# zama-ai/verifiable-fhe-paper

Measured on AMD Instinct MI355X. Metric: vPBS proofs/sec at N=1024 (1/2/4/8 GPU); prover ms/proof vs CPU baseline, higher is better.
Workload: dtype u64; 1 GPU; N=1024 vPBS as IVC chain (BASELINE config 2; verified_pbs ivc_based_vpbs.rs:159-386) via vpbs_ivc_prove_pbs; step = 1 chained proof of the cyclic circuit (2^16 rows) per chain; chains_per_gpu=8, parallelism=replicas, witness=host

## Files before the change

### verifiable-fhe-paper_amd/csrc/hash.hip

```cpp
#include <cstdlib>

#include <algorithm>
#include "kernels.h"
#include "poseidon.h"

namespace vpbs {
namespace {
constexpr unsigned THREADS = 256;

template <bool SAMPLE>
__global__ void __launch_bounds__(THREADS)
leaf_hash_kernel(const u64* __restrict__ lde, unsigned ncols, size_t n_leaves, size_t col_stride, u64* __restrict__ digests,
                 u64* __restrict__ clock_sample) {
    const size_t j = blockIdx.x * (size_t)THREADS + threadIdx.x;
    if (j >= n_leaves) return;
    const bool sample = SAMPLE && clock_sample != nullptr && blockIdx.x == gridDim.x / 2 && threadIdx.x == 0;
    u64 c0 = 0, r0 = 0;
    if (sample) {
        r0 = __builtin_amdgcn_s_memrealtime();
        c0 = __builtin_amdgcn_s_memtime();
    }
    u64 s[12];
#pragma unroll
    for (int i = 0; i < 12; ++i) s[i] = 0;
    if (ncols <= 4) {
#pragma unroll
        for (int k = 0; k < 4; ++k)
            if ((unsigned)k < ncols) s[k] = lde[k * col_stride + j];
    } else {
        u64 nxt[8];
#pragma unroll
        for (int k = 0; k < 8; ++k)
            if ((unsigned)k < ncols) s[k] = lde[(size_t)k * col_stride + j];
        for (unsigned c0 = 0;; c0 += 8) {
            if (c0 + 8 < ncols) {
#pragma unroll
                for (int k = 0; k < 8; ++k)
                    if (c0 + 8 + k < ncols) nxt[k] = lde[(size_t)(c0 + 8 + k) * col_stride + j];
            }
            const bool more = poseidon::permute_sponge(s, ncols - c0, [&](unsigned n) {
#pragma unroll
                for (int k = 0; k < 8; ++k)
                    if ((unsigned)k < n) s[k] = nxt[k];
            });
            if (!more) break;
        }
#pragma unroll
        for (int k = 0; k < 4; ++k) s[k] = gl::canon(s[k]);
    }
    ulonglong2* d = reinterpret_cast<ulonglong2*>(digests + 4 * j);
    d[0] = make_ulonglong2(s[0], s[1]);
    d[1] = make_ulonglong2(s[2], s[3]);
    if (sample) {
        clock_sample[0] = __builtin_amdgcn_s_memtime() - c0;
        clock_sample[1] = __builtin_amdgcn_s_memrealtime() - r0;
    }
}

__global__ void __launch_bounds__(THREADS)
fri_leaf_hash_kernel(const u64* __restrict__ v0, const u64* __restrict__ v1, size_t n_leaves, unsigned arity_bits,
                     u64* __restrict__ digests) {
    const size_t l = blockIdx.x * (size_t)THREADS + threadIdx.x;
    if (l >= n_leaves) return;
    const unsigned arity = 1u << arity_bits;
    const size_t base = l << arity_bits;
    u64 s[12];
#pragma unroll
    for (int i = 0; i < 12; ++i) s[i] = 0;
    if (2 * arity <= 4) {
#pragma unroll
        for (int m = 0; m < 2; ++m)
            if ((unsigned)m < arity) { s[2 * m] = v0[base + m]; s[2 * m + 1] = v1[base + m]; }
    } else {
#pragma unroll
        for (int k = 0; k < 4; ++k)
            if ((unsigned)k < arity) { s[2 * k] = v0[base + k]; s[2 * k + 1] = v1[base + k]; }
        for (unsigned m0 = 0;; m0 += 4) {
            const bool more = poseidon::permute_sponge(s, 2 * (arity - m0), [&](unsigned n) {
#pragma unroll
                for (int k = 0; k < 4; ++k)
                    if (2 * (unsigned)k < n) { s[2 * k] = v0[base + m0 + 4 + k]; s[2 * k + 1] = v1[base + m0 + 4 + k]; }
            });
            if (!more) break;
        }
#pragma unroll
        for (int k = 0; k < 4; ++k) s[k] = gl::canon(s[k]);
    }
    ulonglong2* d = reinterpret_cast<ulonglong2*>(digests + 4 * l);
    d[0] = make_ulonglong2(s[0], s[1]);
    d[1] = make_ulonglong2(s[2], s[3]);
}

__global__ void __launch_bounds__(THREADS)
merkle_level_kernel(const u64* __restrict__ children, u64* __restrict__ parents, size_t n_parents) {
    const size_t i = blockIdx.x * (size_t)THREADS + threadIdx.x;
    if (i >= n_parents) return;
    const ulonglong2* c = reinterpret_cast<const ulonglong2*>(children + 8 * i);
    const ulonglong2 a = c[0], b = c[1], e = c[2], f = c[3];
    u64 s[12] = {a.x, a.y, b.x, b.y, e.x, e.y, f.x, f.y, 0, 0, 0, 0};
// ... 38 lines not shown
            const bool live = i < m;
            u64 x = 0;
            if (live && l < 8) x = k == 0 ? src[8 * i + l] : buf[(k - 1) & 1][8 * i + l];
            x = poseidon::permute_wide(x, lds + g * poseidon::WIDE_LDS_WORDS, l);
            if (live && l < 4) {
                dst[4 * i + l] = x;
                buf[k & 1][4 * i + l] = x;
            }
        }
        __syncthreads();
    }
}

__global__ void __launch_bounds__(THREADS)
fri_leaf_hash_wide_kernel(const u64* __restrict__ v0, const u64* __restrict__ v1, size_t n_leaves, unsigned arity_bits,
                          u64* __restrict__ digests) {
    __shared__ u64 lds[(THREADS / poseidon::WIDE_LANES) * poseidon::WIDE_LDS_WORDS];
    const unsigned l = threadIdx.x & 15, g = threadIdx.x >> 4;
    const size_t leaf = blockIdx.x * (size_t)(THREADS / 16) + g;
    const bool live = leaf < n_leaves;
    const unsigned n_elems = 2u << arity_bits;
    const size_t base = leaf << arity_bits;
    u64 x = 0;
    for (unsigned e0 = 0; e0 < n_elems; e0 += 8) {
        const unsigned e = e0 + l;
        if (l < 8 && e < n_elems && live) x = ((e & 1) ? v1 : v0)[base + (e >> 1)];
        x = poseidon::permute_wide(x, lds + g * poseidon::WIDE_LDS_WORDS, l);
    }
    if (live && l < 4) digests[4 * leaf + l] = x;
}

__global__ void __launch_bounds__(THREADS) permute_batch_kernel(u64* states, size_t n) {
    const size_t i = blockIdx.x * (size_t)THREADS + threadIdx.x;
    if (i >= n) return;
    u64 s[12];
#pragma unroll
    for (int k = 0; k < 12; ++k) s[k] = states[12 * i + k];
    poseidon::permute(s);
#pragma unroll
    for (int k = 0; k < 12; ++k) states[12 * i + k] = s[k];
}

__global__ void __launch_bounds__(THREADS)
hash_rows_kernel(const u64* __restrict__ rows, size_t n, unsigned len, u64* __restrict__ out) {
    const size_t i = blockIdx.x * (size_t)THREADS + threadIdx.x;
    if (i >= n) return;
    const u64* row = rows + i * len;
    u64 s[12];
#pragma unroll
    for (int k = 0; k < 12; ++k) s[k] = 0;
#pragma unroll
    for (int k = 0; k < 8; ++k)
        if ((unsigned)k < len) s[k] = row[k];
    for (unsigned c0 = 0;; c0 += 8) {
        const bool more = poseidon::permute_sponge(s, len - c0, [&](unsigned n) {
#pragma unroll
            for (int k = 0; k < 8; ++k)
                if ((unsigned)k < n) s[k] = row[c0 + 8 + k];
        });
        if (!more) break;
    }
#pragma unroll
    for (int k = 0; k < 4; ++k) out[4 * i + k] = gl::canon(s[k]);
}

struct PowState {
    u64 s[12];
};

__global__ void __launch_bounds__(THREADS)
pow_search_kernel(PowState st, unsigned pos, unsigned pow_bits, u64 start, u64 count, u64 stride, unsigned long long* result) {
    const u64 i = blockIdx.x * (u64)THREADS + threadIdx.x;
    if (i >= stride) return;
    for (u64 off = i; off < count; off += stride) {
        const u64 cand = start + off;
        if (__atomic_load_n(result, __ATOMIC_RELAXED) < cand) return;
        u64 s[12];
#pragma unroll
        for (int k = 0; k < 12; ++k) s[k] = (unsigned)k == pos ? cand : st.s[k];
        poseidon::permute_residues(s);
        if (pow_bits == 0 || (gl::canon(s[7]) >> (64 - pow_bits)) == 0) {
            atomicMin(result, (unsigned long long)cand);
            return;
        }
    }
}
}

void launch_leaf_hash(hipStream_t s, const u64* lde, unsigned ncols, size_t n_leaves, size_t col_stride, u64* digests, u64* clock_sample) {
    if (clock_sample)
        hipLaunchKernelGGL(leaf_hash_kernel<true>, dim3((n_leaves + THREADS - 1) / THREADS), dim3(THREADS), 0, s, lde, ncols, n_leaves,
                           col_stride, digests, clock_sample);
    else
        hipLaunchKernelGGL(leaf_hash_kernel<false>, dim3((n_leaves + THREADS - 1) / THREADS), dim3(THREADS), 0, s, lde, ncols, n_leaves,
                           col_stride, digests, clock_sample);
}
Tuning Tuning::from_env() {
    Tuning t;
    if (const char* e = getenv("VPBS_WIDE_THRESHOLD")) t.wide_threshold = t.fri_leaf_wide_threshold = (size_t)strtoull(e, nullptr, 10);
    if (const char* e = getenv("VPBS_FRI_LEAF_WIDE_THRESHOLD")) t.fri_leaf_wide_threshold = (size_t)strtoull(e, nullptr, 10);
    if (const char* e = getenv("VPBS_MERKLE_CLIMB")) t.merkle_climb = atoi(e) != 0;
    if (const char* e = getenv("VPBS_GATES_FUSED")) t.gates_fused = atoi(e) != 0;
    if (const char* e = getenv("VPBS_GATE_ITEMS")) t.gate_items = (unsigned)std::max(1, atoi(e));
    if (const char* e = getenv("VPBS_GATES_TILE")) t.gates_tile = atoi(e) != 0;
    return t;
}

void launch_fri_leaf_hash(hipStream_t s, const Tuning& tune, const u64* v0, const u64* v1, size_t n_leaves, unsigned arity_bits, u64* digests) {
    if (n_leaves <= tune.fri_leaf_wide_threshold && (2u << arity_bits) > 4) {
        hipLaunchKernelGGL(fri_leaf_hash_wide_kernel, dim3((unsigned)((n_leaves * 16 + THREADS - 1) / THREADS)), dim3(THREADS), 0, s, v0,
                           v1, n_leaves, arity_bits, digests);
        return;
    }
    hipLaunchKernelGGL(fri_leaf_hash_kernel, dim3((n_leaves + THREADS - 1) / THREADS), dim3(THREADS), 0, s, v0, v1, n_leaves,
// ... 49 lines not shown
```

### verifiable-fhe-paper_amd/csrc/poseidon.h

```cpp
#pragma once
#include "gl.h"

namespace poseidon {
using gl::u32;
using gl::u64;

constexpr int WIDTH = 12, RATE = 8, N_ROUNDS = 30, HALF_FULL = 4, N_PARTIAL = 22;

static const u64 RC_HOST[372] = {
#include "poseidon_constants.inc"
};
#if defined(__HIPCC__)
static __constant__ u64 RC_DEV[372] = {
#include "poseidon_constants.inc"
};
#endif

#include "poseidon_partial_groups.inc"
static const PartialGroup PG_HOST[7] = POSEIDON_PARTIAL_GROUPS_INIT;
#if defined(__HIPCC__)
static __constant__ PartialGroup PG_DEV[7] = POSEIDON_PARTIAL_GROUPS_INIT;
#endif
GL_HD const PartialGroup& partial_group(int g) {
#if defined(__HIP_DEVICE_COMPILE__)
// ... 175 lines not shown
            "v_mad_u64_u32 %0, vcc, %10, 39, %0\n\t"
            "v_mad_u64_u32 %1, vcc, %22, 39, %1\n\t"
            "v_mad_u64_u32 %0, vcc, %11, 18, %0\n\t"
            "v_mad_u64_u32 %1, vcc, %23, 18, %1\n\t"
            "v_mad_u64_u32 %0, vcc, %12, 34, %0\n\t"
            "v_mad_u64_u32 %1, vcc, %24, 34, %1\n\t"
            "v_mad_u64_u32 %0, vcc, %13, 20, %0\n\t"
            "v_mad_u64_u32 %1, vcc, %25, 20, %1"
                : "=&v"(acc_lo), "=&v"(acc_hi)
                : POSEIDON_ROW_OPERANDS
                : "vcc");
    }
}
#endif

GL_HD void mds_add_const(u64* s, const u64* kc) {
    u32 lo[12], hi[12];
#pragma unroll
    for (int i = 0; i < 12; ++i) {
        lo[i] = (u32)s[i];
        hi[i] = (u32)(s[i] >> 32);
    }
#pragma unroll
    for (int r = 0; r < 12; ++r) {
        u64 acc_lo, acc_hi;
#if defined(__HIP_DEVICE_COMPILE__)
        u32 xl[12], xh[12];
#pragma unroll
        for (int i = 0; i < 12; ++i) {
            xl[i] = lo[(i + r) % 12];
            xh[i] = hi[(i + r) % 12];
        }
        if (kc) {
            if (r == 0) mds_row<true, true>(xl, xh, kc[r], acc_lo, acc_hi);
            else mds_row<false, true>(xl, xh, kc[r], acc_lo, acc_hi);
        } else {
            if (r == 0) mds_row<true, false>(xl, xh, 0, acc_lo, acc_hi);
            else mds_row<false, false>(xl, xh, 0, acc_lo, acc_hi);
        }
#else
        const u32 C[12] = {17, 15, 41, 16, 2, 28, 13, 13, 39, 18, 34, 20};
        const u64 k = kc ? kc[r] : 0;
        acc_lo = (u32)k, acc_hi = k >> 32;
        for (int i = 0; i < 12; ++i) {
            const u32 c = r == 0 && i == 0 ? C[0] + 8 : C[i];
            acc_lo += (u64)lo[(i + r) % 12] * c;
            acc_hi += (u64)hi[(i + r) % 12] * c;
        }
#endif
        s[r] = fold96(acc_lo, acc_hi);
    }
}

#if defined(__HIP_DEVICE_COMPILE__)
template <unsigned M1>
__device__ __forceinline__ void group_row(u32 d3l, u32 d3h, u32 d2l, u32 d2h, u32 m2, u64 k, const u32* xl, const u32* xh, const u32* m3, u64& acc_lo,
                                          u64& acc_hi) {
    static_assert(M1 <= 64, "inline constant");
    asm("s_mov_b32 s82, %43\n\t"
        "s_and_b32 s83, %44, 0x03ffffff\n\t"
        "s_and_b32 s84, %44, 0xfc000000\n\t"
        "s_mov_b32 s85, 0\n\t"
        "v_mad_u64_u32 %0, vcc, %2, %45, s[82:83]\n\t"
        "v_mad_u64_u32 %1, vcc, %3, %45, s[84:85]\n\t"
        "v_mad_u64_u32 %0, vcc, %4, %6, %0\n\t"
        "v_mad_u64_u32 %1, vcc, %5, %6, %1\n\t"
        "v_mad_u64_u32 %0, vcc, %7, %31, %0\n\t"
        "v_mad_u64_u32 %1, vcc, %19, %31, %1\n\t"
        "v_mad_u64_u32 %0, vcc, %8, %32, %0\n\t"
        "v_mad_u64_u32 %1, vcc, %20, %32, %1\n\t"
        "v_mad_u64_u32 %0, vcc, %9, %33, %0\n\t"
        "v_mad_u64_u32 %1, vcc, %21, %33, %1\n\t"
        "v_mad_u64_u32 %0, vcc, %10, %34, %0\n\t"
        "v_mad_u64_u32 %1, vcc, %22, %34, %1\n\t"
        "v_mad_u64_u32 %0, vcc, %11, %35, %0\n\t"
        "v_mad_u64_u32 %1, vcc, %23, %35, %1\n\t"
        "v_mad_u64_u32 %0, vcc, %12, %36, %0\n\t"
        "v_mad_u64_u32 %1, vcc, %24, %36, %1\n\t"
        "v_mad_u64_u32 %0, vcc, %13, %37, %0\n\t"
        "v_mad_u64_u32 %1, vcc, %25, %37, %1\n\t"
        "v_mad_u64_u32 %0, vcc, %14, %38, %0\n\t"
        "v_mad_u64_u32 %1, vcc, %26, %38, %1\n\t"
        "v_mad_u64_u32 %0, vcc, %15, %39, %0\n\t"
        "v_mad_u64_u32 %1, vcc, %27, %39, %1\n\t"
        "v_mad_u64_u32 %0, vcc, %16, %40, %0\n\t"
        "v_mad_u64_u32 %1, vcc, %28, %40, %1\n\t"
        "v_mad_u64_u32 %0, vcc, %17, %41, %0\n\t"
        "v_mad_u64_u32 %1, vcc, %29, %41, %1\n\t"
        "v_mad_u64_u32 %0, vcc, %18, %42, %0\n\t"
        "v_mad_u64_u32 %1, vcc, %30, %42, %1"
        : "=&v"(acc_lo), "=&v"(acc_hi)
        : "v"(d3l), "v"(d3h), "v"(d2l), "v"(d2h), "s"(m2),
          "v"(xl[0]), "v"(xl[1]), "v"(xl[2]), "v"(xl[3]), "v"(xl[4]), "v"(xl[5]), "v"(xl[6]), "v"(xl[7]), "v"(xl[8]), "v"(xl[9]), "v"(xl[10]),
          "v"(xl[11]),
          "v"(xh[0]), "v"(xh[1]), "v"(xh[2]), "v"(xh[3]), "v"(xh[4]), "v"(xh[5]), "v"(xh[6]), "v"(xh[7]), "v"(xh[8]), "v"(xh[9]), "v"(xh[10]),
          "v"(xh[11]),
          "s"(m3[0]), "s"(m3[1]), "s"(m3[2]), "s"(m3[3]), "s"(m3[4]), "s"(m3[5]), "s"(m3[6]), "s"(m3[7]), "s"(m3[8]), "s"(m3[9]), "s"(m3[10]),
          "s"(m3[11]),
          "s"((u32)k), "s"((u32)(k >> 32)), "n"(M1)
        : "vcc", "scc", "s82", "s83", "s84", "s85");
}
template <int I> struct GroupRow {
    static __device__ __forceinline__ void run(u64* s, const u64* kv, const u32* lo, const u32* hi, u32 d2l, u32 d2h, u32 d3l, u32 d3h) {
        u32 m3[12];
#pragma unroll
        for (int j = 0; j < 12; ++j) m3[j] = MDS3[I][j];
// ... 18 lines not shown
        hi[j] = (u32)(s[j] >> 32);
    }
    u64 a_lo = (u32)k2, a_hi = k2 >> 32;
#pragma unroll
    for (int j = 0; j < 12; ++j) {
        a_lo += (u64)lo[j] * MDS1[0][j];
        a_hi += (u64)hi[j] * MDS1[0][j];
    }
    u64 x2 = fold96(a_lo, a_hi);
    if (GATE || x_out) {
        x2 = gl::canon(x2);
        x_out[0] = x2;
    }
    const u64 d2 = gl::sub_a(sbox(GATE ? w[1] : x2), x2);
    const u32 d2l = (u32)d2, d2h = (u32)(d2 >> 32);
    u64 b_lo = (u32)k3, b_hi = k3 >> 32;
#pragma unroll
    for (int j = 0; j < 12; ++j) {
        b_lo += (u64)lo[j] * MDS2[0][j];
        b_hi += (u64)hi[j] * MDS2[0][j];
    }
    b_lo += (u64)d2l * MDS1[0][0];
    b_hi += (u64)d2h * MDS1[0][0];
    u64 x3 = fold96(b_lo, b_hi);
    if (GATE || x_out) {
        x3 = gl::canon(x3);
        x_out[1] = x3;
    }
    const u64 d3 = gl::sub_a(sbox(GATE ? w[2] : x3), x3);
    const u32 d3l = (u32)d3, d3h = (u32)(d3 >> 32);
#if defined(__HIP_DEVICE_COMPILE__)
    GroupRow<0>::run(s, kv, lo, hi, d2l, d2h, d3l, d3h);
#else
#pragma unroll
    for (int i = 0; i < 12; ++i) {
        const u64 k = kv[i];
        u64 acc_lo = (u32)k, acc_hi = k >> 32;
#pragma unroll
        for (int j = 0; j < 12; ++j) {
            acc_lo += (u64)lo[j] * MDS3[i][j];
            acc_hi += (u64)hi[j] * MDS3[i][j];
        }
        acc_lo += (u64)d2l * MDS2[i][0] + (u64)d3l * MDS1[i][0];
        acc_hi += (u64)d2h * MDS2[i][0] + (u64)d3h * MDS1[i][0];
        s[i] = fold96(acc_lo, acc_hi);
    }
#endif
}
template <bool GATE> GL_HD void partial_group3_core(u64* s, int g, const u64* w, u64* x_out) {
    partial_group3_core<GATE>(s, partial_group(g), w, x_out);
}
GL_HD void partial_group3(u64* s, int g) { partial_group3_core<false>(s, g, nullptr, nullptr); }

static const ClosingGroup CG_HOST = POSEIDON_CLOSING_GROUP_INIT;
#if defined(__HIPCC__)
static __constant__ ClosingGroup CG_DEV = POSEIDON_CLOSING_GROUP_INIT;
#endif
GL_HD const ClosingGroup& closing_group(int z) {
#if defined(__HIP_DEVICE_COMPILE__)
    return (&CG_DEV)[z];
#else
    return (&CG_HOST)[z];
#endif
}
#if defined(__HIP_DEVICE_COMPILE__)
__device__ __forceinline__ void halves_sum(const u32* xl, const u32* xh, u64& sum_lo, u64& sum_hi) {
    asm("v_mad_u64_u32 %0, vcc, %2, 1, 0\n\t"
        "v_mad_u64_u32 %1, vcc, %14, 1, 0\n\t"
        "v_mad_u64_u32 %0, vcc, %3, 1, %0\n\t"
        "v_mad_u64_u32 %1, vcc, %15, 1, %1\n\t"
        "v_mad_u64_u32 %0, vcc, %4, 1, %0\n\t"
        "v_mad_u64_u32 %1, vcc, %16, 1, %1\n\t"
        "v_mad_u64_u32 %0, vcc, %5, 1, %0\n\t"
        "v_mad_u64_u32 %1, vcc, %17, 1, %1\n\t"
        "v_mad_u64_u32 %0, vcc, %6, 1, %0\n\t"
        "v_mad_u64_u32 %1, vcc, %18, 1, %1\n\t"
        "v_mad_u64_u32 %0, vcc, %7, 1, %0\n\t"
        "v_mad_u64_u32 %1, vcc, %19, 1, %1\n\t"
        "v_mad_u64_u32 %0, vcc, %8, 1, %0\n\t"
        "v_mad_u64_u32 %1, vcc, %20, 1, %1\n\t"
        "v_mad_u64_u32 %0, vcc, %9, 1, %0\n\t"
        "v_mad_u64_u32 %1, vcc, %21, 1, %1\n\t"
        "v_mad_u64_u32 %0, vcc, %10, 1, %0\n\t"
        "v_mad_u64_u32 %1, vcc, %22, 1, %1\n\t"
        "v_mad_u64_u32 %0, vcc, %11, 1, %0\n\t"
        "v_mad_u64_u32 %1, vcc, %23, 1, %1\n\t"
        "v_mad_u64_u32 %0, vcc, %12, 1, %0\n\t"
        "v_mad_u64_u32 %1, vcc, %24, 1, %1\n\t"
        "v_mad_u64_u32 %0, vcc, %13, 1, %0\n\t"
        "v_mad_u64_u32 %1, vcc, %25, 1, %1"
        : "=&v"(sum_lo), "=&v"(sum_hi)
        : POSEIDON_ROW_OPERANDS
        : "vcc");
}
template <unsigned M1>
__device__ __forceinline__ void closing_row(u32 d4l, u32 d4h, u32 d3l, u32 d3h, u32 m2, u32 d2l, u32 d2h, u32 m3, u32 tl, u32 th, u32 base, u64 k,
                                            const u32* xl, const u32* xh, const u32* n, u64& acc_lo, u64& acc_hi) {
    static_assert(M1 <= 64, "inline constant");
    asm("s_mov_b32 s82, %49\n\t"
        "s_and_b32 s83, %50, 0x03ffffff\n\t"
        "s_and_b32 s84, %50, 0xfc000000\n\t"
        "s_mov_b32 s85, 0\n\t"
        "v_mad_u64_u32 %0, vcc, %2, %51, s[82:83]\n\t"
        "v_mad_u64_u32 %1, vcc, %3, %51, s[84:85]\n\t"
        "v_mad_u64_u32 %0, vcc, %4, %6, %0\n\t"
        "v_mad_u64_u32 %1, vcc, %5, %6, %1\n\t"
        "v_mad_u64_u32 %0, vcc, %7, %9, %0\n\t"
        "v_mad_u64_u32 %1, vcc, %8, %9, %1\n\t"
        "v_mad_u64_u32 %0, vcc, %10, %12, %0\n\t"
        "v_mad_u64_u32 %1, vcc, %11, %12, %1\n\t"
        "v_mad_u64_u32 %0, vcc, %13, %37, %0\n\t"
        "v_mad_u64_u32 %1, vcc, %25, %37, %1\n\t"
        "v_mad_u64_u32 %0, vcc, %14, %38, %0\n\t"
        "v_mad_u64_u32 %1, vcc, %26, %38, %1\n\t"
        "v_mad_u64_u32 %0, vcc, %15, %39, %0\n\t"
        "v_mad_u64_u32 %1, vcc, %27, %39, %1\n\t"
        "v_mad_u64_u32 %0, vcc, %16, %40, %0\n\t"
// ... 63 lines not shown
    u64 b_lo = (u32)k3, b_hi = k3 >> 32;
#pragma unroll
    for (int j = 0; j < 12; ++j) {
        b_lo += (u64)lo[j] * MDS2[0][j];
        b_hi += (u64)hi[j] * MDS2[0][j];
    }
    b_lo += (u64)d2l * MDS1[0][0];
    b_hi += (u64)d2h * MDS1[0][0];
    const u64 x3 = fold96(b_lo, b_hi);
    const u64 d3 = gl::sub_a(sbox(WIRES ? w[2] : x3), x3);
    const u32 d3l = (u32)d3, d3h = (u32)(d3 >> 32);
    u64 c_lo = (u32)k4, c_hi = k4 >> 32;
#pragma unroll
    for (int j = 0; j < 12; ++j) {
        c_lo += (u64)lo[j] * MDS3[0][j];
        c_hi += (u64)hi[j] * MDS3[0][j];
    }
    c_lo += (u64)d2l * MDS2[0][0] + (u64)d3l * MDS1[0][0];
    c_hi += (u64)d2h * MDS2[0][0] + (u64)d3h * MDS1[0][0];
    const u64 x4 = fold96(c_lo, c_hi);
    const u64 d4 = gl::sub_a(sbox(WIRES ? w[3] : x4), x4);
    const u32 d4l = (u32)d4, d4h = (u32)(d4 >> 32);
    u64 t_lo, t_hi;
#if defined(__HIP_DEVICE_COMPILE__)
    halves_sum(lo, hi, t_lo, t_hi);
#else
    t_lo = 0, t_hi = 0;
    for (int j = 0; j < 12; ++j) {
        t_lo += lo[j];
        t_hi += hi[j];
    }
#endif
    const u64 t = fold96(t_lo, t_hi);
    const u32 tl = (u32)t, th = (u32)(t >> 32);
#if defined(__HIP_DEVICE_COMPILE__)
    ClosingRow<0>::run(s, kv, lo, hi, d2l, d2h, d3l, d3h, d4l, d4h, tl, th);
#else
#pragma unroll
    for (int i = 0; i < 12; ++i) {
        const u64 k = kv[i];
        u64 acc_lo = (u32)k, acc_hi = k >> 32;
#pragma unroll
        for (int j = 0; j < 12; ++j) {
            acc_lo += (u64)lo[j] * (MDS4[i][j] - MDS4_BASE[i]);
            acc_hi += (u64)hi[j] * (MDS4[i][j] - MDS4_BASE[i]);
        }
        acc_lo += (u64)tl * MDS4_BASE[i] + (u64)d2l * MDS3[i][0] + (u64)d3l * MDS2[i][0] + (u64)d4l * MDS1[i][0];
        acc_hi += (u64)th * MDS4_BASE[i] + (u64)d2h * MDS3[i][0] + (u64)d3h * MDS2[i][0] + (u64)d4h * MDS1[i][0];
        s[i] = fold96(acc_lo, acc_hi);
    }
#endif
}
GL_HD void closing_group4(u64* s, int z = 0) { closing_group4_core<false>(s, closing_group(z), nullptr); }

GL_HD void permute_head(u64* s) {
#if defined(__HIP_DEVICE_COMPILE__)
    int z;
    asm volatile("s_mov_b32 %0, 0" : "=s"(z));
#else
    constexpr int z = 0;
#endif
#pragma unroll
    for (int i = 0; i < 12; ++i) s[i] = gl::add_nc(s[i], rc(z + i));
    for (int r = 0; r < HALF_FULL; ++r) {
        u64 kc[12];
#pragma unroll
        for (int i = 0; i < 12; ++i) kc[i] = rc(12 * (r + 1) + i);
#pragma unroll
        for (int i = 0; i < 12; i += 2) sbox2(s[i], s[i + 1]);
        mds_add_const(s, kc);
    }
    {
        for (int g = 0; g < 6; ++g) partial_group3(s, g);
    }
    {
#if defined(__HIP_DEVICE_COMPILE__)
        int z4;
        asm volatile("s_mov_b32 %0, 0" : "=s"(z4));
#else
        constexpr int z4 = 0;
#endif
        closing_group4(s, z4);
    }
    for (int r = HALF_FULL + N_PARTIAL; r < N_ROUNDS - 1; ++r) {
        u64 kc[12];
#pragma unroll
        for (int i = 0; i < 12; ++i) kc[i] = rc(12 * (r + 1) + i);
#pragma unroll
        for (int i = 0; i < 12; i += 2) sbox2(s[i], s[i + 1]);
        mds_add_const(s, kc);
    }
#pragma unroll
    for (int i = 0; i < 12; i += 2) sbox2(s[i], s[i + 1]);
}
struct HeadHalves {
    u32 lo[12], hi[12];
};
GL_HD HeadHalves head_halves(const u64* s) {
    HeadHalves h;
#pragma unroll
    for (int i = 0; i < 12; ++i) {
        h.lo[i] = (u32)s[i];
        h.hi[i] = (u32)(s[i] >> 32);
    }
    return h;
}
template <int FIRST, int COUNT> GL_HD void last_rows(u64* s, const HeadHalves& h) {
    static_assert(FIRST >= 0 && COUNT > 0 && FIRST + COUNT <= 12, "rows of a width-12 state");
#pragma unroll
    for (int r = FIRST; r < FIRST + COUNT; ++r) {
        u64 acc_lo, acc_hi;
#if defined(__HIP_DEVICE_COMPILE__)
        u32 xl[12], xh[12];
#pragma unroll
        for (int i = 0; i < 12; ++i) {
            xl[i] = h.lo[(i + r) % 12];
            xh[i] = h.hi[(i + r) % 12];
        }
        if (r == 0) mds_row<true, false>(xl, xh, 0, acc_lo, acc_hi);
        else mds_row<false, false>(xl, xh, 0, acc_lo, acc_hi);
#else
        const u32 C[12] = {17, 15, 41, 16, 2, 28, 13, 13, 39, 18, 34, 20};
        acc_lo = 0, acc_hi = 0;
        for (int i = 0; i < 12; ++i) {
            const u32 c = r == 0 && i == 0 ? C[0] + 8 : C[i];
            acc_lo += (u64)h.lo[(i + r) % 12] * c;
            acc_hi += (u64)h.hi[(i + r) % 12] * c;
        }
#endif
        s[r] = fold96(acc_lo, acc_hi);
    }
}

GL_HD void permute_residues(u64* s) {
    permute_head(s);
    last_rows<0, 12>(s, head_halves(s));
}
template <class Absorb> GL_HD bool permute_sponge(u64* s, unsigned remaining, Absorb&& absorb) {
    permute_head(s);
#if defined(__HIP_DEVICE_COMPILE__)
    asm volatile("" : "+s"(remaining));
#endif
    const HeadHalves h = head_halves(s);
    if (remaining <= 8) {
        last_rows<0, 4>(s, h);
        return false;
    }
    last_rows<8, 4>(s, h);
    if (remaining < 16) {
        last_rows<0, 8>(s, h);
        absorb(remaining - 8);
    } else {
        absorb(8u);
    }
    return true;
}
GL_HD void permute_digest(u64* s) {
    permute_head(s);
    last_rows<0, 4>(s, head_halves(s));
}
GL_HD void permute(u64* s) {
    permute_residues(s);
#pragma unroll
    for (int i = 0; i < 12; ++i) s[i] = gl::canon(s[i]);
}

#if defined(__HIPCC__)
constexpr int WIDE_LANES = 16, WIDE_LDS_WORDS = 48;
__device__ __forceinline__ u64 permute_wide(u64 x, u64* sh, unsigned l) {
    constexpr u32 C[12] = {17, 15, 41, 16, 2, 28, 13, 13, 39, 18, 34, 20};
    const unsigned row = l < 12 ? l : 0;
    u32 m3[12];
#pragma unroll
    for (int j = 0; j < 12; ++j) m3[j] = MDS3[row][j];
    const u32 m2c = MDS2[row][0], m1c = MDS1[row][0];
    x = gl::add_nc(x, rc(row));
    u64 kplain[9], kgroup[7];
#pragma unroll
    for (int i = 0; i < 9; ++i) {
        const int r = i < 4 ? i : HALF_FULL + N_PARTIAL - 1 + (i - 4);
        kplain[i] = r + 1 < N_ROUNDS ? rc(12 * (r + 1) + row) : 0;
    }
#pragma unroll
    for (int g = 0; g < 7; ++g) kgroup[g] = partial_group(g).kvec[row];
    auto plain_round = [&](u64 k, bool full) {
        if (full || l == 0) x = sbox_ilp(x);
        __builtin_amdgcn_fence(__ATOMIC_ACQ_REL, "wavefront");
        if (l < 12) {
            sh[l] = x;
            sh[l + 12] = x;
        }
        __builtin_amdgcn_fence(__ATOMIC_ACQ_REL, "wavefront");
        u64 al[3] = {(u32)k, 0, 0}, ah[3] = {k >> 32, 0, 0};
#pragma unroll
        for (int i = 0; i < 12; ++i) {
            const u64 v = sh[row + i];
            al[i % 3] += (u64)(u32)v * C[i];
            ah[i % 3] += (v >> 32) * C[i];
        }
        if (l == 0) {
            al[1] += (u64)(u32)x * 8u;
            ah[1] += (x >> 32) * 8u;
        }
        x = fold96(al[0] + al[1] + al[2], ah[0] + ah[1] + ah[2]);
    };
#pragma unroll
    for (int i = 0; i < HALF_FULL; ++i) plain_round(kplain[i], true);
#pragma unroll
    for (int g = 0; g < 7; ++g) {
        const PartialGroup& G = partial_group(g);
        const u64 k2 = G.k2, k3 = G.k3, kv = kgroup[g];
// ... 50 lines not shown
```

### verifiable-fhe-paper_amd/csrc/poseidon_partial_groups.inc

```
static constexpr unsigned MDS1[12][12] = {
    {25, 15, 41, 16, 2, 28, 13, 13, 39, 18, 34, 20},
    {20, 17, 15, 41, 16, 2, 28, 13, 13, 39, 18, 34},
    {34, 20, 17, 15, 41, 16, 2, 28, 13, 13, 39, 18},
    {18, 34, 20, 17, 15, 41, 16, 2, 28, 13, 13, 39},
    {39, 18, 34, 20, 17, 15, 41, 16, 2, 28, 13, 13},
    {13, 39, 18, 34, 20, 17, 15, 41, 16, 2, 28, 13},
    {13, 13, 39, 18, 34, 20, 17, 15, 41, 16, 2, 28},
    {28, 13, 13, 39, 18, 34, 20, 17, 15, 41, 16, 2},
    {2, 28, 13, 13, 39, 18, 34, 20, 17, 15, 41, 16},
    {16, 2, 28, 13, 13, 39, 18, 34, 20, 17, 15, 41},
    {41, 16, 2, 28, 13, 13, 39, 18, 34, 20, 17, 15},
    {15, 41, 16, 2, 28, 13, 13, 39, 18, 34, 20, 17},
};
static constexpr unsigned MDS2[12][12] = {
    {5642, 5952, 4914, 5368, 6238, 5356, 5302, 6080, 5870, 4880, 6818, 5364},
    {5364, 5306, 5832, 4586, 5240, 6222, 5132, 5198, 5976, 5558, 4736, 6546},
    {6818, 5204, 5306, 5832, 4586, 5240, 6222, 5132, 5198, 5976, 5558, 4736},
    {4880, 6546, 5204, 5306, 5832, 4586, 5240, 6222, 5132, 5198, 5976, 5558},
    {5870, 4736, 6546, 5204, 5306, 5832, 4586, 5240, 6222, 5132, 5198, 5976},
    {6080, 5558, 4736, 6546, 5204, 5306, 5832, 4586, 5240, 6222, 5132, 5198},
    {5302, 5976, 5558, 4736, 6546, 5204, 5306, 5832, 4586, 5240, 6222, 5132},
    {5356, 5198, 5976, 5558, 4736, 6546, 5204, 5306, 5832, 4586, 5240, 6222},
    {6238, 5132, 5198, 5976, 5558, 4736, 6546, 5204, 5306, 5832, 4586, 5240},
    {5368, 6222, 5132, 5198, 5976, 5558, 4736, 6546, 5204, 5306, 5832, 4586},
    {4914, 5240, 6222, 5132, 5198, 5976, 5558, 4736, 6546, 5204, 5306, 5832},
    {5952, 4586, 5240, 6222, 5132, 5198, 5976, 5558, 4736, 6546, 5204, 5306},
};
static constexpr unsigned MDS3[12][12] = {
    {1525684, 1438872, 1418228, 1480072, 1422580, 1420320, 1506604, 1416584, 1444108, 1476584, 1436396, 1411808},
    {1411808, 1437100, 1395776, 1375900, 1435272, 1376884, 1375744, 1464500, 1372416, 1394724, 1440536, 1380428},
    {1436396, 1370256, 1445852, 1393568, 1373884, 1442568, 1375940, 1377200, 1473028, 1371072, 1401092, 1440536},
    {1476584, 1379388, 1372080, 1437004, 1389504, 1377372, 1436824, 1374276, 1379280, 1465012, 1371072, 1394724},
    {1444108, 1439776, 1390020, 1371168, 1435324, 1397952, 1377396, 1439008, 1384572, 1379280, 1473028, 1372416},
    {1416584, 1393404, 1439360, 1378892, 1366384, 1437612, 1390568, 1374692, 1439008, 1374276, 1377200, 1464500},
    {1506604, 1367736, 1396108, 1436760, 1377436, 1369088, 1436052, 1390568, 1377396, 1436824, 1375940, 1375744},
    {1420320, 1465780, 1375360, 1395428, 1435544, 1383500, 1369088, 1437612, 1397952, 1377372, 1442568, 1376884},
    {1422580, 1373904, 1463076, 1366432, 1391876, 1435544, 1377436, 1366384, 1435324, 1389504, 1373884, 1435272},
    {1480072, 1374324, 1378912, 1464468, 1366432, 1395428, 1436760, 1378892, 1371168, 1437004, 1393568, 1375900},
    {1418228, 1439872, 1385852, 1378912, 1463076, 1375360, 1396108, 1439360, 1390020, 1372080, 1445852, 1395776},
    {1438872, 1375140, 1439872, 1374324, 1373904, 1465780, 1367736, 1393404, 1439776, 1379388, 1370256, 1437100},
};
struct PartialGroup { unsigned long long kvec[12]; unsigned long long k2, k3; };
#define POSEIDON_PARTIAL_GROUPS_INIT { \
    {{0xfe4e957d77fda909ULL, 0x3847b97fc56907d4ULL, 0x0a1b7d0f67cfc238ULL, 0xc414e2bfdddee685ULL, 0x2717635d4d088529ULL, 0x40491e688918641bULL, 0x560b36b7f479beafULL, 0xda7596d883b42c13ULL, 0xd8b7b84768d7843aULL, 0x733c8ebad2af2843ULL, 0x8f92cf546fb87dcdULL, 0x6081e328cce022cdULL}, 0x7131aa45268d7d8cULL, 0xff1b1d52a1d8bb71ULL}, \
    {{0xd119def35a30b511ULL, 0x6785e26657976c04ULL, 0x4c85e0f0e498b80aULL, 0x09b2f2891e72516eULL, 0xe8b03d4698e681aaULL, 0x943c922624343e1eULL, 0x490186833eb8ae37ULL, 0xab44b27eb875bd36ULL, 0xf675f2dac0d2b4adULL, 0x0735fb41dfb4abedULL, 0xec6d46a358c64e19ULL, 0x71183a53d224b708ULL}, 0x7159cd30c3ac118eULL, 0x50c17f4e8bc2a7b5ULL}, \
    {{0x54eafd5e8c0ef61dULL, 0xfe06121da3b5b838ULL, 0x0ef385ebd5715833ULL, 0x61a0a6709460c24fULL, 0xc6a94f23db583ec5ULL, 0x3bb2b2e7586de7c0ULL, 0xae705460e5c84923ULL, 0x20d3881afc6b4518ULL, 0x0cc8cad7bd42cc91ULL, 0x2f4efc14e6672a3fULL, 0xbd0bae3dce7d33d9ULL, 0xe258d7e08e8bd3b8ULL}, 0x30a4680593258387ULL, 0x875e5dbdfa0a1b6bULL}, \
    {{0x2d5e442f2de9aea9ULL, 0x1c4170bab0c28bfeULL, 0xfbd4c3193585cc9eULL, 0x596c7a704f8f3f2aULL, 0xceef25ac926d22dfULL, 0x54ac7c785c0f4ff3ULL, 0x7c55c7d7dcf17873ULL, 0xdc9e8e30b8caaa76ULL, 0x5f7782ff3c614fcaULL, 0x4d4176f913e999feULL, 0xa5ce4725b751e6f8ULL, 0xf5d10a11c024a67aULL}, 0x775005982d74d7f7ULL, 0xe6b47ac7fadcceacULL}, \
    {{0x5fdb985df94d5f34ULL, 0x3e6e5ea6969897f8ULL, 0x39e628df805fb70aULL, 0x8dabe2e2b77195acULL, 0xbaae0d3685531a78ULL, 0x836cc600e5475c67ULL, 0x6a1cf353276fa432ULL, 0x35f461ba3266eef6ULL, 0xde7afd90ec069d5dULL, 0x5f578ca248341311ULL, 0x606e5560329a8266ULL, 0x88eb2c660628a242ULL}, 0xdd611f1000c17442ULL, 0x82c8567c0dad8fd2ULL}, \
    {{0xbb167cb775013794ULL, 0x87befcca0b83baffULL, 0x44d6d7813828842aULL, 0x3452da396d341fccULL, 0x94b4a33439d5d74fULL, 0xbba4cb68152c5ab5ULL, 0x8798e5ade84f4253ULL, 0x6268ed55dec1949dULL, 0x6084862992f892baULL, 0x3748775cf424ec3fULL, 0x19197866793dcb9fULL, 0xf9cbdd030cb77598ULL}, 0xe89cd854d5d01d33ULL, 0xfc39f87979d52a85ULL}, \
    {{0x3eec5e59c10be794ULL, 0x921c7513b98436fdULL, 0x8f4003a60c2aa013ULL, 0x9f75572964678803ULL, 0x3e9495107539a5e1ULL, 0x617c7acbc1db897fULL, 0x43530ee6648e366aULL, 0xce98d5d027df583fULL, 0xb6d54eb500e52d7cULL, 0x553fc8926939fc86ULL, 0x30cfbdbb7b960c7fULL, 0xfa93f9bc7bf7381aULL}, 0xde122bebe9a39368ULL, 0x5718e9d82e27faebULL}, \
}
static constexpr unsigned MDS4[12][12] = {
    {381558488, 369288112, 374533544, 369959168, 369454632, 373358944, 370265576, 368886800, 375007320, 369607648, 370277912, 373854368},
    {373854368, 357623704, 358824096, 362304040, 357790720, 359163384, 361468960, 358453864, 358738272, 362530840, 358873600, 358107144},
    {370277912, 363385904, 359530600, 358628928, 362580520, 359632512, 359263656, 362413968, 360578840, 358445408, 364635672, 358873600},
    {369607648, 357841672, 363242464, 357426104, 357304992, 362611176, 357965408, 358508792, 362402336, 358324552, 358445408, 362530840},
    {375007320, 358891216, 359772456, 363367680, 358082088, 359247008, 363011304, 359184368, 360706264, 362402336, 360578840, 358738272},
    {368886800, 362336792, 358838416, 357739464, 361725808, 357942552, 357503856, 362032872, 359184368, 358508792, 362413968, 358453864},
    {370265576, 357418192, 363216664, 357590848, 357148184, 362702816, 357138904, 357503856, 363011304, 357965408, 359263656, 361468960},
    {373358944, 358888936, 358959456, 362859992, 357846656, 358765576, 362702816, 357942552, 359247008, 362611176, 359632512, 359163384},
    {369454632, 360921296, 359059288, 357057728, 361200024, 357846656, 357148184, 361725808, 358082088, 357304992, 362580520, 357790720},
    {369959168, 358531384, 362427136, 358297672, 357057728, 362859992, 357590848, 357739464, 363367680, 357426104, 358628928, 362304040},
    {374533544, 359211952, 360256728, 362427136, 359059288, 358959456, 363216664, 358838416, 359772456, 363242464, 359530600, 358824096},
    {369288112, 362193128, 359211952, 358531384, 360921296, 358888936, 357418192, 362336792, 358891216, 357841672, 363385904, 357623704},
};
static constexpr unsigned MDS4_BASE[12] = {368886800, 357623704, 358445408, 357304992, 358082088, 357503856, 357138904, 357846656, 357057728, 357057728, 358824096, 357418192};
struct ClosingGroup { unsigned long long kvec[12]; unsigned long long k2, k3, k4; };
#define POSEIDON_CLOSING_GROUP_INIT {{0xdc95f1ec2eb3244dULL, 0x287446500cf761ecULL, 0x8b0d2dd37a860ec8ULL, 0xc5f62d4d042a566cULL, 0xc10a7d2f956ec953ULL, 0x435e1e18c9743ccdULL, 0x9f0b0c6ef65b1a78ULL, 0x776d3954f3c88850ULL, 0x0dea5a60554b6830ULL, 0x53ae1b1b1753161bULL, 0x82f6927bdb4b82b4ULL, 0x5b176968ca1309e4ULL}, 0xde122bebe9a39368ULL, 0x5718e9d82e27faebULL, 0x3eec5e59c10be794ULL}
```

Baseline: 0.2134 vPBS proofs/s.

## Specialize Poseidon first round for zero capacity and regroup partial rounds by four

```diff
diff --git a/verifiable-fhe-paper_amd/csrc/hash.hip b/verifiable-fhe-paper_amd/csrc/hash.hip
--- a/verifiable-fhe-paper_amd/csrc/hash.hip
+++ b/verifiable-fhe-paper_amd/csrc/hash.hip
@@ -32,19 +32,20 @@
 #pragma unroll
         for (int k = 0; k < 8; ++k)
             if ((unsigned)k < ncols) s[k] = lde[(size_t)k * col_stride + j];
-        for (unsigned c0 = 0;; c0 += 8) {
-            if (c0 + 8 < ncols) {
-#pragma unroll
-                for (int k = 0; k < 8; ++k)
-                    if (c0 + 8 + k < ncols) nxt[k] = lde[(size_t)(c0 + 8 + k) * col_stride + j];
-            }
-            const bool more = poseidon::permute_sponge(s, ncols - c0, [&](unsigned n) {
+        poseidon::sponge_from_zero(
+            s, ncols,
+            [&](unsigned c) {
+                if (c < ncols) {
+#pragma unroll
+                    for (int k = 0; k < 8; ++k)
+                        if (c + k < ncols) nxt[k] = lde[(size_t)(c + k) * col_stride + j];
+                }
+            },
+            [&](unsigned, unsigned n) {
 #pragma unroll
                 for (int k = 0; k < 8; ++k)
                     if ((unsigned)k < n) s[k] = nxt[k];
             });
-            if (!more) break;
-        }
 #pragma unroll
         for (int k = 0; k < 4; ++k) s[k] = gl::canon(s[k]);
     }
@@ -189,14 +190,13 @@
 #pragma unroll
     for (int k = 0; k < 8; ++k)
         if ((unsigned)k < len) s[k] = row[k];
-    for (unsigned c0 = 0;; c0 += 8) {
-        const bool more = poseidon::permute_sponge(s, len - c0, [&](unsigned n) {
+    poseidon::sponge_from_zero(
+        s, len, [](unsigned) {},
+        [&](unsigned w, unsigned n) {
 #pragma unroll
             for (int k = 0; k < 8; ++k)
-                if ((unsigned)k < n) s[k] = row[c0 + 8 + k];
+                if ((unsigned)k < n) s[k] = row[w + k];
         });
-        if (!more) break;
-    }
 #pragma unroll
     for (int k = 0; k < 4; ++k) out[4 * i + k] = gl::canon(s[k]);
 }
diff --git a/verifiable-fhe-paper_amd/csrc/poseidon.h b/verifiable-fhe-paper_amd/csrc/poseidon.h
--- a/verifiable-fhe-paper_amd/csrc/poseidon.h
+++ b/verifiable-fhe-paper_amd/csrc/poseidon.h
@@ -251,6 +251,78 @@
     }
 }
 
+static const u64 ZC_K1_HOST[12] = POSEIDON_ZERO_CAPACITY_K1_INIT;
+#if defined(__HIPCC__)
+static __constant__ u64 ZC_K1_DEV[12] = POSEIDON_ZERO_CAPACITY_K1_INIT;
+#endif
+GL_HD u64 zero_capacity_k1(int i) {
+#if defined(__HIP_DEVICE_COMPILE__)
+    return ZC_K1_DEV[i];
+#else
+    return ZC_K1_HOST[i];
+#endif
+}
+#if defined(__HIP_DEVICE_COMPILE__)
+template <int R> __device__ __forceinline__ void mds_row8(const u32* xl, const u32* xh, u64 k, u64& acc_lo, u64& acc_hi) {
+    asm("s_mov_b32 s82, %18\n\t"
+        "s_and_b32 s83, %19, 0x03ffffff\n\t"
+        "s_and_b32 s84, %19, 0xfc000000\n\t"
+        "s_mov_b32 s85, 0\n\t"
+        "v_mad_u64_u32 %0, vcc, %2, %20, s[82:83]\n\t"
+        "v_mad_u64_u32 %1, vcc, %10, %20, s[84:85]\n\t"
+        "v_mad_u64_u32 %0, vcc, %3, %21, %0\n\t"
+        "v_mad_u64_u32 %1, vcc, %11, %21, %1\n\t"
+        "v_mad_u64_u32 %0, vcc, %4, %22, %0\n\t"
+        "v_mad_u64_u32 %1, vcc, %12, %22, %1\n\t"
+        "v_mad_u64_u32 %0, vcc, %5, %23, %0\n\t"
+        "v_mad_u64_u32 %1, vcc, %13, %23, %1\n\t"
+        "v_mad_u64_u32 %0, vcc, %6, %24, %0\n\t"
+        "v_mad_u64_u32 %1, vcc, %14, %24, %1\n\t"
+        "v_mad_u64_u32 %0, vcc, %7, %25, %0\n\t"
+        "v_mad_u64_u32 %1, vcc, %15, %25, %1\n\t"
+        "v_mad_u64_u32 %0, vcc, %8, %26, %0\n\t"
+        "v_mad_u64_u32 %1, vcc, %16, %26, %1\n\t"
+        "v_mad_u64_u32 %0, vcc, %9, %27, %0\n\t"
+        "v_mad_u64_u32 %1, vcc, %17, %27, %1"
+        : "=&v"(acc_lo), "=&v"(acc_hi)
+        : "v"(xl[0]), "v"(xl[1]), "v"(xl[2]), "v"(xl[3]), "v"(xl[4]), "v"(xl[5]), "v"(xl[6]), "v"(xl[7]),
+          "v"(xh[0]), "v"(xh[1]), "v"(xh[2]), "v"(xh[3]), "v"(xh[4]), "v"(xh[5]), "v"(xh[6]), "v"(xh[7]),
+          "s"((u32)k), "s"((u32)(k >> 32)),
+          "n"(MDS1[R][0]), "n"(MDS1[R][1]), "n"(MDS1[R][2]), "n"(MDS1[R][3]), "n"(MDS1[R][4]), "n"(MDS1[R][5]), "n"(MDS1[R][6]),
+          "n"(MDS1[R][7])
+        : "vcc", "scc", "s82", "s83", "s84", "s85");
+}
+template <int R> struct MdsRow8 {
+    static_assert(MDS1[R][0] <= 64 && MDS1[R][7] <= 64, "inline constants");
+    static __device__ __forceinline__ void run(u64* s, const u64* kc, const u32* lo, const u32* hi) {
+        u64 acc_lo, acc_hi;
+        mds_row8<R>(lo, hi, kc[R], acc_lo, acc_hi);
+        s[R] = fold96(acc_lo, acc_hi);
+        if constexpr (R + 1 < 12) MdsRow8<R + 1>::run(s, kc, lo, hi);
+    }
+};
+#endif
+GL_HD void mds8_add_const(u64* s, const u64* kc) {
+    u32 lo[8], hi[8];
+#pragma unroll
+    for (int j = 0; j < 8; ++j) {
+        lo[j] = (u32)s[j];
+        hi[j] = (u32)(s[j] >> 32);
+    }
+#if defined(__HIP_DEVICE_COMPILE__)
+    MdsRow8<0>::run(s, kc, lo, hi);
+#else
+    for (int i = 0; i < 12; ++i) {
+        u64 acc_lo = (u32)kc[i], acc_hi = kc[i] >> 32;
+        for (int j = 0; j < 8; ++j) {
+            acc_lo += (u64)lo[j] * MDS1[i][j];
+            acc_hi += (u64)hi[j] * MDS1[i][j];
+        }
+        s[i] = fold96(acc_lo, acc_hi);
+    }
+#endif
+}
+
 #if defined(__HIP_DEVICE_COMPILE__)
 template <unsigned M1>
 __device__ __forceinline__ void group_row(u32 d3l, u32 d3h, u32 d2l, u32 d2h, u32 m2, u64 k, const u32* xl, const u32* xh, const u32* m3, u64& acc_lo,
@@ -375,17 +447,18 @@
 }
 GL_HD void partial_group3(u64* s, int g) { partial_group3_core<false>(s, g, nullptr, nullptr); }
 
-static const ClosingGroup CG_HOST = POSEIDON_CLOSING_GROUP_INIT;
+static const ClosingGroup G4_HOST[POSEIDON_N_GROUPS4] = POSEIDON_GROUPS4_INIT;
 #if defined(__HIPCC__)
-static __constant__ ClosingGroup CG_DEV = POSEIDON_CLOSING_GROUP_INIT;
-#endif
-GL_HD const ClosingGroup& closing_group(int z) {
-#if defined(__HIP_DEVICE_COMPILE__)
-    return (&CG_DEV)[z];
-#else
-    return (&CG_HOST)[z];
-#endif
-}
+static __constant__ ClosingGroup G4_DEV[POSEIDON_N_GROUPS4] = POSEIDON_GROUPS4_INIT;
+#endif
+GL_HD const ClosingGroup& group4_constants(int g) {
+#if defined(__HIP_DEVICE_COMPILE__)
+    return G4_DEV[g];
+#else
+    return G4_HOST[g];
+#endif
+}
+GL_HD const ClosingGroup& closing_group(int z) { return group4_constants(POSEIDON_N_GROUPS4 - 1 + z); }
 #if defined(__HIP_DEVICE_COMPILE__)
 __device__ __forceinline__ void halves_sum(const u32* xl, const u32* xh, u64& sum_lo, u64& sum_hi) {
     asm("v_mad_u64_u32 %0, vcc, %2, 1, 0\n\t"
@@ -555,8 +628,14 @@
 #endif
 }
 GL_HD void closing_group4(u64* s, int z = 0) { closing_group4_core<false>(s, closing_group(z), nullptr); }
-
-GL_HD void permute_head(u64* s) {
+GL_HD void partial_group4(u64* s, int g) {
+    closing_group4_core<false>(s, group4_constants(g), nullptr);
+#if defined(__HIP_DEVICE_COMPILE__)
+    asm volatile("" : "+v"(s[0]), "+v"(s[1]), "+v"(s[2]), "+v"(s[3]), "+v"(s[4]), "+v"(s[5]), "+v"(s[6]), "+v"(s[7]), "+v"(s[8]), "+v"(s[9]), "+v"(s[10]), "+v"(s[11]));
+#endif
+}
+
+GL_HD void head_first_constants(u64* s) {
 #if defined(__HIP_DEVICE_COMPILE__)
     int z;
     asm volatile("s_mov_b32 %0, 0" : "=s"(z));
@@ -565,7 +644,34 @@
 #endif
 #pragma unroll
     for (int i = 0; i < 12; ++i) s[i] = gl::add_nc(s[i], rc(z + i));
-    for (int r = 0; r < HALF_FULL; ++r) {
+}
+GL_HD void head_zero_capacity_round(u64* s) {
+    u64 kc[12];
+#pragma unroll
+    for (int i = 0; i < 12; ++i) kc[i] = zero_capacity_k1(i);
+#pragma unroll
+    for (int i = 0; i < 8; ++i) s[i] = gl::add_nc(s[i], rc(i));
+#pragma unroll
+    for (int i = 0; i < 8; i += 2) sbox2(s[i], s[i + 1]);
+    mds8_add_const(s, kc);
+}
+GL_HD void partial_rounds(u64* s) {
+#pragma nounroll
+    for (int g = 0; g < POSEIDON_N_GROUPS4 - 1; ++g) partial_group4(s, g);
+#pragma nounroll
+    for (int g = 4; g < 6; ++g) partial_group3(s, g);
+    {
+#if defined(__HIP_DEVICE_COMPILE__)
+        int z4;
+        asm volatile("s_mov_b32 %0, 0" : "=s"(z4));
+#else
+        constexpr int z4 = 0;
+#endif
+        closing_group4(s, z4);
+    }
+}
+GL_HD void head_from_round(u64* s, int r0) {
+    for (int r = r0; r < HALF_FULL; ++r) {
         u64 kc[12];
 #pragma unroll
         for (int i = 0; i < 12; ++i) kc[i] = rc(12 * (r + 1) + i);
@@ -573,18 +679,7 @@
         for (int i = 0; i < 12; i += 2) sbox2(s[i], s[i + 1]);
         mds_add_const(s, kc);
     }
-    {
-        for (int g = 0; g < 6; ++g) partial_group3(s, g);
-    }
-    {
-#if defined(__HIP_DEVICE_COMPILE__)
-        int z4;
-        asm volatile("s_mov_b32 %0, 0" : "=s"(z4));
-#else
-        constexpr int z4 = 0;
-#endif
-        closing_group4(s, z4);
-    }
+    partial_rounds(s);
     for (int r = HALF_FULL + N_PARTIAL; r < N_ROUNDS - 1; ++r) {
         u64 kc[12];
 #pragma unroll
@@ -595,6 +690,15 @@
     }
 #pragma unroll
     for (int i = 0; i < 12; i += 2) sbox2(s[i], s[i + 1]);
+}
+template <bool ZERO_CAPACITY = false> GL_HD void permute_head(u64* s) {
+    if constexpr (ZERO_CAPACITY) {
+        head_zero_capacity_round(s);
+        head_from_round(s, 1);
+    } else {
+        head_first_constants(s);
+        head_from_round(s, 0);
+    }
 }
 struct HeadHalves {
     u32 lo[12], hi[12];
@@ -639,8 +743,7 @@
     permute_head(s);
     last_rows<0, 12>(s, head_halves(s));
 }
-template <class Absorb> GL_HD bool permute_sponge(u64* s, unsigned remaining, Absorb&& absorb) {
-    permute_head(s);
+template <class Absorb> GL_HD bool sponge_rows(u64* s, unsigned remaining, Absorb&& absorb) {
 #if defined(__HIP_DEVICE_COMPILE__)
     asm volatile("" : "+s"(remaining));
 #endif
@@ -658,8 +761,23 @@
     }
     return true;
 }
+template <bool FIRST = false, class Absorb> GL_HD bool permute_sponge(u64* s, unsigned remaining, Absorb&& absorb) {
+    permute_head<FIRST>(s);
+    return sponge_rows(s, remaining, absorb);
+}
+template <class Prefetch, class Absorb> GL_HD void sponge_from_zero(u64* s, unsigned n_words, Prefetch&& prefetch, Absorb&& absorb) {
+    head_zero_capacity_round(s);
+    int r0 = 1;
+    for (unsigned w = 0;; w += 8) {
+        prefetch(w + 8);
+        head_from_round(s, r0);
+        if (!sponge_rows(s, n_words - w, [&](unsigned n) { absorb(w + 8, n); })) break;
+        head_first_constants(s);
+        r0 = 0;
+    }
+}
 GL_HD void permute_digest(u64* s) {
-    permute_head(s);
+    permute_head<true>(s);
     last_rows<0, 4>(s, head_halves(s));
 }
 GL_HD void permute(u64* s) {
diff --git a/verifiable-fhe-paper_amd/csrc/poseidon_partial_groups.inc b/verifiable-fhe-paper_amd/csrc/poseidon_partial_groups.inc
--- a/verifiable-fhe-paper_amd/csrc/poseidon_partial_groups.inc
+++ b/verifiable-fhe-paper_amd/csrc/poseidon_partial_groups.inc
@@ -66,4 +66,11 @@
 };
 static constexpr unsigned MDS4_BASE[12] = {368886800, 357623704, 358445408, 357304992, 358082088, 357503856, 357138904, 357846656, 357057728, 357057728, 358824096, 357418192};
 struct ClosingGroup { unsigned long long kvec[12]; unsigned long long k2, k3, k4; };
-#define POSEIDON_CLOSING_GROUP_INIT {{0xdc95f1ec2eb3244dULL, 0x287446500cf761ecULL, 0x8b0d2dd37a860ec8ULL, 0xc5f62d4d042a566cULL, 0xc10a7d2f956ec953ULL, 0x435e1e18c9743ccdULL, 0x9f0b0c6ef65b1a78ULL, 0x776d3954f3c88850ULL, 0x0dea5a60554b6830ULL, 0x53ae1b1b1753161bULL, 0x82f6927bdb4b82b4ULL, 0x5b176968ca1309e4ULL}, 0xde122bebe9a39368ULL, 0x5718e9d82e27faebULL, 0x3eec5e59c10be794ULL}
+constexpr int POSEIDON_N_GROUPS4 = 4;
+#define POSEIDON_GROUPS4_INIT { \
+    {{0xf98c67d1df07db89ULL, 0x09d2e43296235ec6ULL, 0xbe81163a6e92c550ULL, 0xf230521b33206e6cULL, 0x1d72f688ab68cfc8ULL, 0x8ff9191a3fa28552ULL, 0x3bec05e3d159f5f9ULL, 0x75f144dea73c9a0dULL, 0x8c0c7ce1adee3131ULL, 0x5dc5350a28851016ULL, 0x1311a633b9bca949ULL, 0xcd31a8d40fa722edULL}, 0x7131aa45268d7d8cULL, 0xff1b1d52a1d8bb71ULL, 0xfe4e957d77fda909ULL}, \
+    {{0xac07d226c0346861ULL, 0xbabc45d6bdddb41fULL, 0x695c781222d4edcfULL, 0x74a1f01ef7e988ffULL, 0xc380181869e42148ULL, 0xf8b7633b06b03c8aULL, 0x52c95b7716425e94ULL, 0x7db8389bce0dbca9ULL, 0x66318aa79f7bb8e6ULL, 0x9caca242f00bc7e8ULL, 0x2e417238f3005989ULL, 0x1a74daac1acc7c24ULL}, 0xdcef0797c2b69ec7ULL, 0xfd13809b6947306dULL, 0x4ab94850f8a340c1ULL}, \
+    {{0x00d0476b7909352bULL, 0xa389c715bb997a27ULL, 0xde88b6cd063b374dULL, 0x63b42e220f78e0a7ULL, 0xa5ad5ee1a1496db2ULL, 0x7559ae8ba2e1c381ULL, 0x250fd08eccba67aaULL, 0x6950ac4fad906213ULL, 0x81d88fbeb743e437ULL, 0xa0d1511ca7bd55a6ULL, 0x8cb3e89bc108530bULL, 0x3d9057dd15e026c6ULL}, 0x5a3f1bb1c53a9645ULL, 0xd6f59155762e0a3dULL, 0xd523d9b689e183cfULL}, \
+    {{0xdc95f1ec2eb3244dULL, 0x287446500cf761ecULL, 0x8b0d2dd37a860ec8ULL, 0xc5f62d4d042a566cULL, 0xc10a7d2f956ec953ULL, 0x435e1e18c9743ccdULL, 0x9f0b0c6ef65b1a78ULL, 0x776d3954f3c88850ULL, 0x0dea5a60554b6830ULL, 0x53ae1b1b1753161bULL, 0x82f6927bdb4b82b4ULL, 0x5b176968ca1309e4ULL}, 0xde122bebe9a39368ULL, 0x5718e9d82e27faebULL, 0x3eec5e59c10be794ULL}, \
+}
+#define POSEIDON_ZERO_CAPACITY_K1_INIT {0x62cfea8e55341db8ULL, 0x53ae0d422f8cc6efULL, 0xac29b888aeef84d6ULL, 0x90cc491f71b5fd4eULL, 0x638cd97d1f14244cULL, 0xf3fc76291302124dULL, 0xc57293658eb53e57ULL, 0x60bea017e5f8e6a2ULL, 0x54c44c3971082de9ULL, 0xb7d39352c39511f2ULL, 0xb39c19ddc44cc469ULL, 0x301a0d485cf527f6ULL}
```

After: 0.2113 vPBS proofs/s, median of 2. No clear change (-1.0%).
